# Terascale-All-sensing-Research-Studio/MOV-SLAM

Measured on AMD Instinct MI355X. Metric: local-BA iterations/sec (50 KF x 20k MapPoint window), higher is better.
Workload: dtype f64; 1 GPU; LocalBundleAdjustment 50 KF + 10 fixed x 20000 MapPoints, E=110510 mono edges, Huber on, 10 LM iterations (cfg3, seed 1003); one window per GPU; parallelism=1 window

## Files before the change

### mov-slam_amd/csrc/structure.cpp

```cpp
#include "structure.h"

#include <algorithm>
#include <cstdlib>
#include <cstring>

namespace movba {

void reset_structure(Structure& s, int NP, int P, int E)
{
    s.nfree = 0; s.npairs = 0; s.nitems = 0; s.max_degree = 0; s.nentries = 0; s.already_grouped = true; s.n_fixed = 0; s.n_agg = 0; s.reordered = false;
    s.free_pose.clear(); s.pair_i.clear(); s.pair_j.clear(); s.items.clear(); s.sched.clear(); s.sched_per_xcd = 0; s.row_ent.clear();
    s.cblk_g.clear(); s.cblk_h.clear(); s.cblk_ptr.clear(); s.cblk_ent.clear(); s.ent_i.clear(); s.ent_j.clear(); s.ent_l.clear(); s.E_free = 0;
    s.NP = NP; s.P = P; s.E = E;
}

void index_poses(const uint8_t* pose_fixed, Structure& s)
{
    const int NP = s.NP;
    s.hidx.assign(NP, -1);
    std::vector<int32_t>& pstart = s.pose_slot0;
    pstart.assign(NP + 1, -1);
    int run = 0;
    for (int i = 0; i < NP; ++i) {
        if (pose_fixed[i]) { s.n_fixed++; continue; }
        if (s.pose_edges[i] > 0) { s.hidx[i] = s.nfree++; s.free_pose.push_back(i); pstart[i] = run; run += s.pose_edges[i]; }
    }
// ... 86 lines not shown
                --pos;
            }
            fe_h[pos] = h; fe_g[pos] = g;
            if (pos > base && fe_h[pos - 1] == h) return MOVBA_ERR_ARG;
            if (pos + 1 < fe_h.size() && fe_h[pos + 1] == h) return MOVBA_ERR_ARG;
        }
        fe_start[l + 1] = (int32_t)fe_h.size();
    }
    return MOVBA_OK;
}

int finish_pairs(Structure& s, const int32_t* cnt)
{
    const int nf = s.nfree;
    s.pid.assign((size_t)nf * (size_t)nf, -1);
    s.pair_i.clear(); s.pair_j.clear();
    for (int i = 0; i < nf; ++i) { s.pid[(size_t)i * nf + i] = i; s.pair_i.push_back(i); s.pair_j.push_back(i); }
    for (int i = 0; i < nf; ++i)
        for (int j = i + 1; j < nf; ++j)
            if (cnt[(size_t)i * nf + j] > 0) {
                s.pid[(size_t)i * nf + j] = (int32_t)s.pair_i.size();
                s.pair_i.push_back(i); s.pair_j.push_back(j);
            }
    s.npairs = (int)s.pair_i.size();
    s.pair_ptr.assign(s.npairs + 1, 0);
    for (int p = 0; p < s.npairs; ++p) s.pair_ptr[p + 1] = s.pair_ptr[p] + cnt[(size_t)s.pair_i[p] * nf + s.pair_j[p]];
    s.nentries = s.pair_ptr[s.npairs];
    if (s.nentries > (int64_t)0x7fffffff) return MOVBA_ERR_ARG;
    if (nf > 0 && s.pair_ptr[nf] != (int64_t)s.E_free) return MOVBA_ERR_ARG;

    s.items.clear();
    s.pair_item_start.assign(s.npairs + 1, 0);
    for (int p = 0; p < s.npairs; ++p) {
        const int64_t cap = p < nf ? kSchurChunkDiag : kSchurChunk, len = s.pair_ptr[p + 1] - s.pair_ptr[p];
        const int64_t parts = (len + cap - 1) / cap;
        const int64_t chunk = parts > 0 ? ((len + parts - 1) / parts + 3) / 4 * 4 : cap;
        s.pair_item_start[p] = (int32_t)s.items.size();
        for (int64_t b = s.pair_ptr[p]; b < s.pair_ptr[p + 1]; b += chunk)
            s.items.push_back(Item{ p, (int32_t)b, (int32_t)std::min<int64_t>(b + chunk, s.pair_ptr[p + 1]), p < nf ? 1 : 0 });
    }
    s.pair_item_start[s.npairs] = (int32_t)s.items.size();
    s.nitems = (int)s.items.size();

    {
        const int ipw = kSchurWaves / kSchurWPI;
        std::vector<int32_t>& order = s.tmp_order;
        order.resize(s.nitems);
        {
            int n = 0, od = nf < s.npairs ? s.pair_item_start[nf] : s.nitems;
            for (int i = 0; i < nf; ++i) {
                for (int k = s.pair_item_start[i]; k < s.pair_item_start[i + 1]; ++k) order[n++] = k;
                while (od < s.nitems && s.pair_i[s.items[od].pair] == i) order[n++] = od++;
            }
        }
        auto weight = [&](int k) { const Item& it = s.items[k]; return (int64_t)(it.end - it.begin) * (it.diag ? 3 : 2) + 128; };
        int64_t total = 0;
        for (int k = 0; k < s.nitems; ++k) total += weight(k);
        std::vector<uint64_t>& key = s.tmp_key;
        key.resize(s.nitems);
        int seg_begin[9];
        {
            int64_t acc = 0; int x = 0;
            seg_begin[0] = 0;
            for (int n = 0; n < s.nitems; ++n) {
                while (x < 7 && acc >= (total * (x + 1)) / 8) seg_begin[++x] = n;
                const int64_t wgt = weight(order[n]);
                key[n] = ((uint64_t)(0x7fffffff - wgt) << 32) | (uint32_t)n;
                acc += wgt;
            }
            while (x < 8) seg_begin[++x] = s.nitems;
        }
#ifndef MOVBA_SCHUR_T1
#define MOVBA_SCHUR_T1 128
#define MOVBA_SCHUR_T2 256
#endif
#ifndef MOVBA_SCHUR_DW
#define MOVBA_SCHUR_DW 4
#endif
        auto waves_of = [&](int k) { const Item& it = s.items[k]; const int n = it.end - it.begin; return it.diag ? MOVBA_SCHUR_DW : (n > MOVBA_SCHUR_T2 ? 4 : (n > MOVBA_SCHUR_T1 ? 2 : 1)); };
        size_t longest = 1;
        for (int g = 0; g < 8; ++g) {
            std::sort(key.begin() + seg_begin[g], key.begin() + seg_begin[g + 1]);
            size_t slots = 0;
            for (int n = seg_begin[g]; n < seg_begin[g + 1]; ++n) {
                const size_t nw = (size_t)waves_of(order[(uint32_t)key[n]]);
                if ((slots & 3) + nw > 4) slots = (slots + 3) & ~(size_t)3;
                slots += nw;
            }
            longest = std::max(longest, (slots + 3) & ~(size_t)3);
        }
        (void)ipw;
        s.sched_per_xcd = (int)longest;
        s.sched.assign((size_t)8 * s.sched_per_xcd, SchedItem{ 0, 0, -1, 0, 0, -1, -1, 0 });
        for (int g = 0; g < 8; ++g) {
            size_t slots = 0;
            for (int n = seg_begin[g]; n < seg_begin[g + 1]; ++n) {
                const int item = order[(uint32_t)key[n]];
                const Item& it = s.items[item];
                const int nw = waves_of(item);
                if ((slots & 3) + (size_t)nw > 4) slots = (slots + 3) & ~(size_t)3;
                const int len = it.end - it.begin, epw = (len + nw - 1) / nw;
                for (int sub = 0; sub < nw; ++sub) {
                    const int wb = std::min(it.begin + sub * epw, it.end), we = std::min(wb + epw, it.end);
                    s.sched[(size_t)g * s.sched_per_xcd + slots + sub] = SchedItem{ wb, we, (item << 1) | (it.diag ? 1 : 0),
                                                                                   s.free_pose[s.pair_i[it.pair]], s.free_pose[s.pair_j[it.pair]], -1, -1, sub | (nw << 8) };
                }
                slots += (size_t)nw;
            }
        }
    }

    {
        s.row_ptr.assign(nf + 1, 0);
        for (int p = 0; p < s.npairs; ++p) {
            s.row_ptr[s.pair_i[p] + 1]++;
            if (p >= nf) s.row_ptr[s.pair_j[p] + 1]++;
        }
        for (int i = 0; i < nf; ++i) s.row_ptr[i + 1] = s.row_ptr[i] + ((s.row_ptr[i + 1] + 1) & ~1);
        s.row_ent.assign((size_t)s.row_ptr[nf], RowEnt{ -1, 0, 0, 0 });
        std::vector<int32_t>& cur = s.tmp_order;
        cur.assign(s.row_ptr.begin(), s.row_ptr.begin() + nf);
        for (int p = nf; p < s.npairs; ++p) s.row_ent[cur[s.pair_j[p]]++] = RowEnt{ p, s.pair_i[p], 1, 0 };
        for (int i = 0; i < nf; ++i) s.row_ent[cur[i]++] = RowEnt{ i, i, 0, 0 };
        for (int p = nf; p < s.npairs; ++p) s.row_ent[cur[s.pair_i[p]]++] = RowEnt{ p, s.pair_j[p], 0, 0 };
    }
    return MOVBA_OK;
}

bool covisibility_order(int nf, const int32_t* cnt, std::vector<int32_t>& new_of_old)
{
    new_of_old.resize(nf);
    for (int i = 0; i < nf; ++i) new_of_old[i] = i;
    if (nf < 3) return false;
    auto linked = [&](int a, int b) { return a == b ? false : (a < b ? cnt[(size_t)a * nf + b] : cnt[(size_t)b * nf + a]) > 0; };
    std::vector<int32_t> deg(nf, 0);
    for (int i = 0; i < nf; ++i) for (int j = i + 1; j < nf; ++j) if (cnt[(size_t)i * nf + j] > 0) { deg[i]++; deg[j]++; }
    auto envelope = [&](const std::vector<int32_t>& old_of_new) {
        int64_t env = 0;
        for (int r = 0; r < nf; ++r) {
            int first = r;
            for (int c = 0; c < r; ++c) if (linked(old_of_new[r], old_of_new[c])) { first = c; break; }
            env += r - first;
        }
        return env;
    };
    std::vector<int32_t> order, level(nf), queue;
    std::vector<uint8_t> placed(nf, 0);
    auto bfs = [&](int root, std::vector<int32_t>& out) {
        out.clear(); out.push_back(root);
        std::fill(level.begin(), level.end(), -1); level[root] = 0;
        for (size_t h = 0; h < out.size(); ++h) {
            const int v = out[h];
            const size_t first = out.size();
            for (int u = 0; u < nf; ++u) if (!placed[u] && level[u] < 0 && linked(v, u)) { level[u] = level[v] + 1; out.push_back(u); }
            std::sort(out.begin() + first, out.end(), [&](int a, int b) { return deg[a] != deg[b] ? deg[a] < deg[b] : a < b; });
        }
        return level[out.back()];
    };
    order.reserve(nf);
    for (;;) {
        int root = -1;
        for (int i = 0; i < nf; ++i) if (!placed[i] && (root < 0 || deg[i] < deg[root])) root = i;
        if (root < 0) break;
        for (int sweep = 0; sweep < 2; ++sweep) {
            const int depth = bfs(root, queue);
            int far = -1;
            for (int v : queue) if (level[v] == depth && (far < 0 || deg[v] < deg[far])) far = v;
            if (far == root) break;
            root = far;
        }
        bfs(root, queue);
        for (int v : queue) { placed[v] = 1; order.push_back(v); }
    }
    std::reverse(order.begin(), order.end());
    std::vector<int32_t> natural(nf);
    for (int i = 0; i < nf; ++i) natural[i] = i;
    const int64_t env_nat = envelope(natural), env_rcm = envelope(order);
    if (!(env_rcm * 5 < env_nat * 4)) return false;
    for (int k = 0; k < nf; ++k) new_of_old[order[k]] = k;
    return true;
}

void apply_pose_order(Structure& s, const std::vector<int32_t>& new_of_old, int32_t* cnt)
{
    const int nf = s.nfree;
    std::vector<int32_t> fp(nf);
    for (int h = 0; h < nf; ++h) fp[new_of_old[h]] = s.free_pose[h];
    s.free_pose = fp;
    for (int h = 0; h < nf; ++h) s.hidx[s.free_pose[h]] = h;
    int run = 0;
    for (int h = 0; h < nf; ++h) { s.pose_slot0[s.free_pose[h]] = run; run += s.pose_edges[s.free_pose[h]]; }
    if (cnt) {
        std::vector<int32_t> c2((size_t)nf * nf, 0);
        for (int i = 0; i < nf; ++i)
            for (int j = i; j < nf; ++j) {
                const int a = new_of_old[i], b = new_of_old[j];
                c2[(size_t)std::min(a, b) * nf + std::max(a, b)] = cnt[(size_t)i * nf + j];
            }
        std::memcpy(cnt, c2.data(), sizeof(int32_t) * c2.size());
    }
}

int build_structure(const movba_lba_desc& d, Structure& s)
{
    const int rc = build_basic(d, s);
    if (rc != MOVBA_OK) return rc;
    const int P = s.P, nf = s.nfree;

    std::vector<int32_t> fe_start, fe_h, fe_g;
    const int rf = free_lists(s, fe_start, fe_h, fe_g);
    if (rf != MOVBA_OK) return rf;
    std::vector<int32_t> cnt((size_t)nf * (size_t)nf, 0);
    for (int l = 0; l < P; ++l)
        for (int a = fe_start[l]; a < fe_start[l + 1]; ++a) {
            int32_t *row = &cnt[(size_t)fe_h[a] * nf];
            for (int b = a; b < fe_start[l + 1]; ++b) row[fe_h[b]]++;
        }
    if (nf <= 80 && !s.no_reorder) {
        std::vector<int32_t> new_of_old;
        if (covisibility_order(nf, cnt.data(), new_of_old)) {
            apply_pose_order(s, new_of_old, nullptr);
            build_slots(s);
            const int rf2 = free_lists(s, fe_start, fe_h, fe_g);
            if (rf2 != MOVBA_OK) return rf2;
            std::fill(cnt.begin(), cnt.end(), 0);
            for (int l = 0; l < P; ++l)
                for (int a = fe_start[l]; a < fe_start[l + 1]; ++a) {
                    int32_t *row = &cnt[(size_t)fe_h[a] * nf];
                    for (int b = a; b < fe_start[l + 1]; ++b) row[fe_h[b]]++;
                }
            s.reordered = true;
        }
    }
    const int rp = finish_pairs(s, cnt.data());
    if (rp != MOVBA_OK) return rp;
// ... 8 lines not shown
                const int32_t *prow = &s.pid[(size_t)fe_h[a] * nf];
                const int32_t ga = fe_g[a];
                for (int b = a + 1; b < fe_start[l + 1]; ++b) {
                    const int32_t pos = cur[prow[fe_h[b]]]++;
                    s.ent_i[pos] = s.slot[ga]; s.ent_j[pos] = s.slot[fe_g[b]]; s.ent_l[pos] = l;
                }
            }
    }
    return MOVBA_OK;
}

void build_coarse(Structure& s, const int32_t* agg_row0, int n_agg)
{
    const int nf = s.nfree, G = n_agg;
    s.n_agg = G;
    s.cblk_g.clear(); s.cblk_h.clear(); s.cblk_ent.clear(); s.cblk_ij.clear(); s.cblk_ptr.assign(1, 0);
    s.multi_pairs.clear();
    for (int p = nf; p < s.npairs; ++p)
        if (s.pair_item_start[p + 1] - s.pair_item_start[p] > 1) s.multi_pairs.push_back(p);
    std::vector<int32_t> agg_of(nf, 0);
    for (int g = 0; g < G; ++g)
        for (int i = agg_row0[g]; i < agg_row0[g + 1]; ++i) agg_of[i] = g;
    std::vector<std::vector<int32_t>> lists((size_t)G * G), ijs((size_t)G * G);
    for (int i = 0; i < nf; ++i)
        for (int e = s.row_ptr[i]; e < s.row_ptr[i + 1]; ++e)
            if (s.row_ent[e].block >= 0) {
                const size_t b = (size_t)agg_of[i] * G + agg_of[s.row_ent[e].col];
                const int pr = s.row_ent[e].block;
                const bool single = pr >= nf && s.pair_item_start[pr + 1] - s.pair_item_start[pr] == 1;
                const int src_idx = single ? s.pair_item_start[pr] : pr;
                lists[b].push_back((src_idx << 2) | (s.row_ent[e].transposed ? 2 : 0) | (single ? 1 : 0));
                ijs[b].push_back((i << 16) | s.row_ent[e].col);
            }
    for (int g = 0; g < G; ++g)
        for (int h = 0; h < G; ++h) {
            const std::vector<int32_t>& l = lists[(size_t)g * G + h];
            if (l.empty()) continue;
            s.cblk_g.push_back(g); s.cblk_h.push_back(h);
            s.cblk_ent.insert(s.cblk_ent.end(), l.begin(), l.end());
            s.cblk_ij.insert(s.cblk_ij.end(), ijs[(size_t)g * G + h].begin(), ijs[(size_t)g * G + h].end());
            s.cblk_ptr.push_back((int32_t)s.cblk_ent.size());
        }
}

}
```

### mov-slam_amd/csrc/structure.h

```cpp
#pragma once
#include <cstdint>
#include <vector>

#include "movba.h"

namespace movba {

struct Int2 { int32_t x, y; };
struct Int4 { int32_t x, y, z, w; };
struct Item { int32_t pair, begin, end, diag; };
struct SchedItem {
    int32_t begin, end, tag , pose_i, pose_j ;
    int32_t dst_a, dst_b;
    int32_t sub;
};
struct RowEnt { int32_t block, col, transposed, pad; };

struct Structure {
    int NP = 0, P = 0, E = 0, nfree = 0;
    int npairs = 0, nitems = 0, max_degree = 0;
    int64_t nentries = 0;
    bool already_grouped = true;
    bool reordered = false;
    bool no_reorder = false;
    int n_fixed = 0;
    std::vector<int32_t> hidx;
    std::vector<int32_t> free_pose;
    std::vector<int32_t> perm;
    std::vector<int32_t> tmp_order; std::vector<uint64_t> tmp_key;
    std::vector<int32_t> pose_edges, pose_slot0;
    std::vector<int32_t> pt_start;
    std::vector<int32_t> g_pose, g_point;
    const int32_t *gp = nullptr, *gl = nullptr;
    std::vector<int32_t> pair_i, pair_j;
    std::vector<int32_t> pair_item_start;
    std::vector<int64_t> pair_ptr;
    std::vector<int32_t> pid;
    std::vector<int32_t> slot;
    std::vector<int32_t> ent_i, ent_j, ent_l;
    int E_free = 0;
    std::vector<Item> items;
    std::vector<SchedItem> sched;
    int sched_per_xcd = 0;
    std::vector<int32_t> row_ptr;
// ... 15 lines not shown
#ifndef MOVBA_SCHUR_EPW_DIAG
#define MOVBA_SCHUR_EPW_DIAG 128
#endif
constexpr int kSchurWaves = MOVBA_SCHUR_WAVES;
constexpr int kSchurWPI = MOVBA_SCHUR_WPI;
constexpr int kSchurChunkDiag = MOVBA_SCHUR_EPW_DIAG * kSchurWPI;
constexpr int kSchurChunk = MOVBA_SCHUR_EPW * kSchurWPI;

int build_structure(const movba_lba_desc& d, Structure& s);
int build_basic(const movba_lba_desc& d, Structure& s, int32_t* rank_out = nullptr);
void reset_structure(Structure& s, int NP, int P, int E);
void index_poses(const uint8_t* pose_fixed, Structure& s);
void build_slots(Structure& s);
int finish_pairs(Structure& s, const int32_t* cnt);

bool covisibility_order(int nf, const int32_t* cnt, std::vector<int32_t>& new_of_old);
void apply_pose_order(Structure& s, const std::vector<int32_t>& new_of_old, int32_t* cnt );

}
```

### mov-slam_amd/csrc/upload.cpp

```cpp
#include <algorithm>
#include <cmath>
#include <cstring>
#include <vector>

#include "handle.h"
#include "kernels.h"

using namespace movba;

namespace {

inline void put(void *dst, const void *src, size_t bytes) { if (bytes) std::memcpy(dst, src, bytes); }

struct EdgeLayout {
    size_t gpose = 0, ptstart = 0, hidx = 0;
    size_t a_end = 0;
    size_t gpoint = 0, free_pose = 0, slot = 0;
    size_t base = 0;
    size_t raw_begin = 0, obs = 0, isig = 0, obsr = 0, pose0 = 0, point0 = 0, kcam = 0;
    size_t grouped_end = 0;
    size_t perm = 0;
    size_t max_end = 0;
    bool has_kcam = false;
};
// ... 88 lines not shown
    int32_t seq = 0;
    StructDev sd{};
    bool dev_structure = false, ent_packed = false, filled_early = false;
    bool scan_pending = false;
    bool sorted_structure = false;
    size_t s2_off = 0, s2_keys_in = 0, s2_keys_out = 0, s2_vals_in = 0, s2_tmp = 0, s2_tmp_bytes = 0;
    uint64_t fill_gen = 0;
    size_t noff = 0, o_ent = 0, o_slotpt = 0;
    size_t pair_begin = 0, hole = 0, h2d = 0, total = 0;
    size_t o_items = 0, o_sched = 0, o_pi = 0, o_pj = 0, o_pis = 0, o_rowptr = 0, o_rowent = 0, o_plan = 0;
    size_t o_cg = 0, o_ch = 0, o_cp = 0, o_ce = 0, o_cij = 0, o_multi = 0, o_pid = 0, o_prange = 0, o_dtp = 0, o_dtk = 0;
    size_t o_st[2][11] = {};
    size_t o_obspm = 0, o_obsrpm = 0, o_part = 0, o_blocks = 0, o_blocks_ov = 0, o_blocks_c = 0, o_aci = 0, o_acitag = 0;
    size_t o_bp = 0, o_xp = 0, o_scale = 0, o_hmax = 0, o_tick = 0, o_recd = 0, o_imgb = 0, o_ctrl = 0, o_chi2 = 0, o_outl = 0;
    size_t o_dtiles = 0, o_ddiag = 0, o_dfail = 0, o_dx = 0, o_dflags = 0, o_dcontrib = 0, o_dstamps = 0;
    std::vector<int32_t> lane_plan;
    int rec_slots = 1;
    size_t ncb = 0;
    int ntile = 0;
    bool dense_one = false, dense_stamps = false;
    double t0 = 0.0, lap_t = 0.0;
    bool lap_on = false;

    Upload(movba_handle *h_, const movba_lba_desc *d_) : h(h_), d(d_), NP(d_->n_poses), P(d_->n_points), E(d_->n_edges) {}
    ~Upload() { h->packer.wait(); if (direct_raw && !raw_synced) (void)hipStreamSynchronize(h->copy_stream); }

    const Structure &s() const { return h->st; }
    void lap(const char *what)
    {
        if (!lap_on) return;
        const double t = now_ms();
// ... 338 lines not shown
    if (!s().already_grouped) {
        { const int rw = join_helper(); if (rw) return rw; }
        HIP_TRY(hipStreamWaitEvent(h->stream, h->copy_event, 0));
        HIP_TRY(hipMemcpyAsync(h->arena + L.raw_begin, sg + L.raw_begin, edge_bytes - L.raw_begin, hipMemcpyHostToDevice, h->stream));
    }
    edge_b_queued = true;
    return MOVBA_OK;
}

int Upload::structure_on_host()
{
    const int rc = build_structure(*d, h->st);
    if (rc < 0) return rc;
    rank_mode = false;
    pack_b(false); edge_b_stale = true;
    noff = (size_t)(s().nentries - s().E_free);
    o_slotpt = c.take<int32_t>((size_t)s().E_free + 1);
    return MOVBA_OK;
}

int Upload::carve_scratch(bool basic)
{
    const int nchunks = (P + 63) / 64;
    Carver sc;
    so_cnt = sc.take<int32_t>(nbins); so_err = sc.take<int32_t>(4);
    so_pe = sc.take<int32_t>(basic ? NP : 0); so_info = sc.take<int32_t>(basic ? kBasicInfo : 0);
    so_ent0 = sc.take<int32_t>(nbins);
    so_cntw = sc.take<int32_t>(sorted_structure ? 0 : (size_t)nbins * nchunks);
    so_cntpt = sc.take<int32_t>(sorted_structure ? (size_t)P + 1 : 0);
    so_fixed = sc.take<uint8_t>(basic ? (size_t)NP + 4 : 0);
// ... 60 lines not shown
{
    int rc = carve_scratch(false); if (rc) return rc;
    HIP_TRY(hipMemsetAsync(h->scratch.p + so_cnt, 0, so_err + 16 - so_cnt, h->stream));
    rc = launch_counts(); if (rc) return rc;
    lap("edge H2D + count launches");
    return after_counts();
}

int Upload::after_counts()
{
    int32_t *cnt = misc();
    if (!dev_first) { const int rc = wait_for_counts(); if (rc) return rc; }
    if (cnt[nbins] != 0) return MOVBA_ERR_ARG;
    lap("wait for the pair counts");
    if (!h->st.no_reorder) {
        std::vector<int32_t> new_of_old;
        if (covisibility_order(nf, cnt, new_of_old)) {
            apply_pose_order(h->st, new_of_old, cnt);
            h->st.reordered = true;
            std::memcpy(sg + L.hidx, s().hidx.data(), sizeof(int32_t) * NP);
            std::memcpy(sg + L.base, s().pose_slot0.data(), sizeof(int32_t) * NP);
            std::memcpy(sg + L.free_pose, s().free_pose.data(), sizeof(int32_t) * nf);
            HIP_TRY(hipMemcpyAsync(h->arena + L.hidx, sg + L.hidx, sizeof(int32_t) * NP, hipMemcpyHostToDevice, h->stream));
            if (dev_first) {
                HIP_TRY(hipMemcpyAsync(h->arena + L.base, sg + L.base, sizeof(int32_t) * NP, hipMemcpyHostToDevice, h->stream));
                HIP_TRY(hipMemcpyAsync(h->arena + L.free_pose, sg + L.free_pose, sizeof(int32_t) * nf, hipMemcpyHostToDevice, h->stream));
            } else edge_b_stale = true;
            HIP_TRY(hipMemsetAsync(h->scratch.p + so_cnt, 0, so_err + 16 - so_cnt, h->stream));
            HIP_TRY(launch_struct_count(sd, h->stream));
            HIP_TRY(launch_struct_counts_out(sd, nullptr, 0, h->stream));
            HIP_TRY(launch_struct_scan(sd, h->stream));
            scan_pending = false;
// ... 147 lines not shown
        const bool forced = h->opt.solver == 2 || (h->opt.solver == 0 && band_env == 1);
        const bool off = h->opt.solver == 3 || h->opt.solver == 1 || (h->opt.solver == 0 && band_env == 0);
        const bool want = forced || (h->rows_kernel && est <= 130000.0);
        h->band = want && !off && band_supported(nf, bw);
    }
    if (h->rows_kernel && !h->band) build_coarse(h->st, h->pp.wave_row0, kPcgRowsThreads / 64);
    lap("pcg plan + coarse lists");
}

int Upload::lay_out_rest()
{
    pair_begin = c.off; hole = pair_begin - L.max_end;
    o_items = c.take<Item>((size_t)s().nitems + 1); o_sched = c.take<SchedItem>(s().sched.size() + 1);
    o_pi = c.take<int32_t>(s().npairs + 1); o_pj = c.take<int32_t>(s().npairs + 1); o_pis = c.take<int32_t>(s().npairs + 1);
    o_rowptr = c.take<int32_t>(nf + 1); o_rowent = c.take<RowEnt>(s().row_ent.size() + 1);
    lane_plan.clear();
    if (h->rows_kernel) {
        lane_plan.assign((size_t)kPcgRowsThreads * 12, -1);
        for (int wv = 0; wv < kPcgRowsThreads / 64; ++wv) {
            const int r0 = h->pp.wave_row0[wv], r1 = h->pp.wave_row0[wv + 1];
            const int P0 = s().row_ptr[r0] >> 1, P1 = s().row_ptr[r1] >> 1;
            for (int ln = 0; ln < 64 && P0 + ln < P1; ++ln)
                for (int k = 0; k < 2; ++k) {
                    const RowEnt &re = s().row_ent[2 * (P0 + ln) + k];
                    int32_t *pl = &lane_plan[((size_t)(wv * 64 + ln) * 3 + k) * 4];
                    if (re.block < 0) continue;
                    pl[0] = re.block; pl[1] = (re.col * 6) | (re.transposed ? (1 << 30) : 0);
                    pl[2] = s().pair_item_start[re.block]; pl[3] = s().pair_item_start[re.block + 1];
                }
            for (int ln = 0; ln < 64; ++ln) {
// ... 2 lines not shown
                if (ln >= 6 * (r1 - r0)) continue;
                const int bi = r0 + ln / 6;
                pl[0] = s().pair_item_start[bi]; pl[1] = s().pair_item_start[bi + 1]; pl[2] = s().row_ptr[bi]; pl[3] = s().row_ptr[bi + 1];
            }
        }
        for (int wv = 0; wv <= kPcgRowsThreads / 64; ++wv) h->pp.wave_ent0[wv] = s().row_ptr[h->pp.wave_row0[wv]];
        h->pp.nrowent = s().row_ptr[nf];
    }
    rec_slots = 1;
    for (int hh = 0; hh < nf; ++hh) rec_slots = std::max(rec_slots, (int)(s().pair_item_start[hh + 1] - s().pair_item_start[hh]));
    for (SchedItem &si : h->st.sched) {
        si.dst_a = -1; si.dst_b = -1;
        if (si.tag >= 0 && (si.tag & 1)) { const Item &it = s().items[(size_t)(si.tag >> 1)]; si.dst_a = it.pair * rec_slots + ((si.tag >> 1) - s().pair_item_start[it.pair]); }
    }
    if (h->rows_kernel && !h->pp.overflow) {
        std::vector<int32_t> slot_of_item((size_t)s().nitems, -1);
        for (size_t q = 0; q < s().sched.size(); ++q)
            if (s().sched[q].tag >= 0 && (s().sched[q].sub & 0xff) == 0) slot_of_item[(size_t)(s().sched[q].tag >> 1)] = (int32_t)q;
        for (int t = 0; t < kPcgRowsThreads; ++t)
            for (int k = 0; k < 2; ++k) {
                const int32_t *pl = &lane_plan[((size_t)t * 3 + k) * 4];
                if (pl[0] < nf || pl[3] - pl[2] != 1) continue;
                SchedItem &si = h->st.sched[(size_t)slot_of_item[(size_t)pl[2]]];
                const int32_t dst = 36 * k * kPcgRowsThreads + t;
                if ((pl[1] >> 30) & 1) si.dst_b = dst; else si.dst_a = dst;
            }
    }
    ncb = s().cblk_g.size();
    o_plan = c.take<int32_t>(lane_plan.size() + 4);
    o_cg = c.take<int32_t>(ncb + 1); o_ch = c.take<int32_t>(ncb + 1); o_cp = c.take<int32_t>(ncb + 2); o_ce = c.take<int32_t>(s().cblk_ent.size() + 1);
    o_cij = c.take<int32_t>(s().cblk_ij.size() + 1); o_multi = c.take<int32_t>(s().multi_pairs.size() + 1);
    o_pid = c.take<int32_t>((size_t)nf * nf + 1);
    ntile = dense_ntile(nf);
// ... 6 lines not shown
    if (!dev_structure) o_ent = c.take<int32_t>(ent_words());
    h2d = c.off;
    if (!state_carved) carve_state();
    const size_t part_stride = ((size_t)s().nitems * kPartStride + 31) / 32 * 32;
    o_part = c.take<double>(part_stride + 1); o_blocks = c.take<double>((size_t)s().npairs * 36 + 1);
    o_recd = c.take<double>((size_t)nf * rec_slots * 48 + 2); o_imgb = c.take<double>((size_t)72 * kPcgRowsThreads);
    o_blocks_ov = c.take<double>(h->rows_kernel && h->pp.overflow ? s().row_ent.size() * 36 + 2 : 2);
    o_blocks_c = c.take<double>((size_t)s().npairs * 36 + 1);
    o_dtiles = c.take<double>(dense_tiles_doubles(nf)); o_ddiag = c.take<double>((size_t)ntile * kDenseNB * kDenseNB + 1); o_dfail = c.take<int32_t>(4);
    o_dx = c.take<double>((size_t)ntile * kDenseNB + 1);
    o_dflags = c.take<uint32_t>(dense_one ? (size_t)dense_flag_words(ntile) : 8);
    o_dcontrib = c.take<double>(dense_one ? (size_t)ntile * ntile * kDenseNB : 1);
    dense_stamps = process_switches().dense_stamps;
    o_dstamps = c.take<unsigned long long>(dense_one && dense_stamps ? 6 * h->dplan.tasks.size() : 1);
    total = c.off;

    if (total > h->arena_cap || h2d - hole + misc_bytes > h->stage_cap) { const int rw = join_helper(); if (rw) return rw; }
    int rc = ensure_arena(h, total); if (rc) return rc;
    if (dev_first && (h->arena_gen != arena_gen_at_edge_copy || h2d - hole + misc_bytes > h->stage_cap)) return kRetryClassic;
    if (h->arena_gen != arena_gen_at_edge_copy) {
        HIP_TRY(hipMemcpyAsync(h->arena, sg, edge_bytes, hipMemcpyHostToDevice, h->stream));
        aim_struct_dev();
    }
    if (h2d - hole + misc_bytes > h->stage_cap) {
        rc = ensure_stage(h, h2d - hole + misc_bytes); if (rc) return rc;
        sg = h->stage;
        pack_edges(true);
    }
    return MOVBA_OK;
}
// ... 5 lines not shown
        if (ent_packed) {
            unsigned long long *e64 = reinterpret_cast<unsigned long long *>(eh);
            for (size_t k = 0; k < noff; ++k) e64[k] = ent_pack(s().ent_i[k], s().ent_j[k], s().ent_l[k]);
        } else {
            put(eh, s().ent_i.data(), sizeof(int32_t) * noff); put(eh + noff, s().ent_j.data(), sizeof(int32_t) * noff);
            put(eh + 2 * noff, s().ent_l.data(), sizeof(int32_t) * noff);
        }
    }
    put(sp(o_items), s().items.data(), sizeof(Item) * (size_t)s().nitems);
    put(sp(o_sched), s().sched.data(), sizeof(SchedItem) * s().sched.size());
    put(sp(o_pi), s().pair_i.data(), sizeof(int32_t) * s().npairs);
    put(sp(o_pj), s().pair_j.data(), sizeof(int32_t) * s().npairs);
    put(sp(o_pis), s().pair_item_start.data(), sizeof(int32_t) * (s().npairs + 1));
    put(sp(o_rowptr), s().row_ptr.data(), sizeof(int32_t) * (nf + 1));
    put(sp(o_rowent), s().row_ent.data(), sizeof(RowEnt) * s().row_ent.size());
    if (!lane_plan.empty()) put(sp(o_plan), lane_plan.data(), sizeof(int32_t) * lane_plan.size());
    put(sp(o_cg), s().cblk_g.data(), sizeof(int32_t) * ncb);
    put(sp(o_ch), s().cblk_h.data(), sizeof(int32_t) * ncb);
    put(sp(o_cp), s().cblk_ptr.data(), sizeof(int32_t) * s().cblk_ptr.size());
    put(sp(o_ce), s().cblk_ent.data(), sizeof(int32_t) * s().cblk_ent.size());
    put(sp(o_cij), s().cblk_ij.data(), sizeof(int32_t) * s().cblk_ij.size());
    put(sp(o_multi), s().multi_pairs.data(), sizeof(int32_t) * s().multi_pairs.size());
    put(sp(o_pid), s().pid.data(), sizeof(int32_t) * (size_t)nf * nf);
    if (dense_one) {
        put(sp(o_dtp), h->dplan.task_ptr.data(), sizeof(int32_t) * h->dplan.task_ptr.size());
        put(sp(o_dtk), h->dplan.tasks.data(), sizeof(DenseTask) * h->dplan.tasks.size());
        int32_t *pr = reinterpret_cast<int32_t *>(sp(o_prange));
        for (size_t q = 0; q < (size_t)nf * nf; ++q) {
            const int32_t pair = s().pid[q];
            pr[2 * q] = pair >= 0 ? s().pair_item_start[pair] : 0;
            pr[2 * q + 1] = pair >= 0 ? s().pair_item_start[pair + 1] : 0;
        }
    }
    lap("carve + pack pair region");
}

int Upload::send_pairs()
{
    const double t2 = now_ms();
    h->prof.structure_ms += (t2 - t0) - upload_host_ms;
    if (h2d - pair_begin <= (size_t)1 << 20) {
        IngestArgs ia{};
        ia.seg[0] = IngestSeg{ h->stage_dev + L.max_end, h->arena + pair_begin, ((h2d - pair_begin) + 3) & ~(size_t)3 };
        ia.nseg = 1; ia.counter = nullptr; ia.wait_for = 0;
        HIP_TRY(launch_ingest(ia, h->stream));
    } else
        HIP_TRY(hipMemcpyAsync(h->arena + pair_begin, sg + L.max_end, h2d - pair_begin, hipMemcpyHostToDevice, h->stream));
    if (!(filled_early && fill_gen == h->arena_gen)) { const int rq = queue_slots_and_fill(); if (rq) return rq; }
    { const int rw = join_helper(); if (rw) return rw; }
// ... 153 lines not shown
```

Baseline: 9478 LM iterations/s.

## Speed up host-side structure build with radix sort, adjacency-list RCM and reused scratch

```diff
diff --git a/mov-slam_amd/csrc/structure.cpp b/mov-slam_amd/csrc/structure.cpp
--- a/mov-slam_amd/csrc/structure.cpp
+++ b/mov-slam_amd/csrc/structure.cpp
@@ -9,7 +9,7 @@
 void reset_structure(Structure& s, int NP, int P, int E)
 {
     s.nfree = 0; s.npairs = 0; s.nitems = 0; s.max_degree = 0; s.nentries = 0; s.already_grouped = true; s.n_fixed = 0; s.n_agg = 0; s.reordered = false;
-    s.free_pose.clear(); s.pair_i.clear(); s.pair_j.clear(); s.items.clear(); s.sched.clear(); s.sched_per_xcd = 0; s.row_ent.clear();
+    s.free_pose.clear(); s.pair_i.clear(); s.pair_j.clear(); s.items.clear(); s.sched_per_xcd = 0; s.row_ent.clear();
     s.cblk_g.clear(); s.cblk_h.clear(); s.cblk_ptr.clear(); s.cblk_ent.clear(); s.ent_i.clear(); s.ent_j.clear(); s.ent_l.clear(); s.E_free = 0;
     s.NP = NP; s.P = P; s.E = E;
 }
@@ -126,61 +126,102 @@
 {
     const int nf = s.nfree;
     s.pid.assign((size_t)nf * (size_t)nf, -1);
-    s.pair_i.clear(); s.pair_j.clear();
-    for (int i = 0; i < nf; ++i) { s.pid[(size_t)i * nf + i] = i; s.pair_i.push_back(i); s.pair_j.push_back(i); }
-    for (int i = 0; i < nf; ++i)
-        for (int j = i + 1; j < nf; ++j)
-            if (cnt[(size_t)i * nf + j] > 0) {
-                s.pid[(size_t)i * nf + j] = (int32_t)s.pair_i.size();
-                s.pair_i.push_back(i); s.pair_j.push_back(j);
-            }
-    s.npairs = (int)s.pair_i.size();
-    s.pair_ptr.assign(s.npairs + 1, 0);
+    s.pair_i.resize((size_t)nf * (nf + 1) / 2); s.pair_j.resize((size_t)nf * (nf + 1) / 2);
+    {
+        int32_t *pi = s.pair_i.data(), *pj = s.pair_j.data(), *pid = s.pid.data();
+        for (int i = 0; i < nf; ++i) { pid[(size_t)i * nf + i] = i; pi[i] = i; pj[i] = i; }
+        int np = nf;
+        for (int i = 0; i < nf; ++i) {
+            const int32_t *row = cnt + (size_t)i * nf;
+            int32_t *prow = pid + (size_t)i * nf;
+            for (int j = i + 1; j < nf; ++j)
+                if (row[j] > 0) { prow[j] = np; pi[np] = i; pj[np] = j; ++np; }
+        }
+        s.npairs = np;
+        s.pair_i.resize(np); s.pair_j.resize(np);
+    }
+    s.pair_ptr.resize(s.npairs + 1);
+    s.pair_ptr[0] = 0;
     for (int p = 0; p < s.npairs; ++p) s.pair_ptr[p + 1] = s.pair_ptr[p] + cnt[(size_t)s.pair_i[p] * nf + s.pair_j[p]];
     s.nentries = s.pair_ptr[s.npairs];
     if (s.nentries > (int64_t)0x7fffffff) return MOVBA_ERR_ARG;
     if (nf > 0 && s.pair_ptr[nf] != (int64_t)s.E_free) return MOVBA_ERR_ARG;
 
-    s.items.clear();
-    s.pair_item_start.assign(s.npairs + 1, 0);
-    for (int p = 0; p < s.npairs; ++p) {
-        const int64_t cap = p < nf ? kSchurChunkDiag : kSchurChunk, len = s.pair_ptr[p + 1] - s.pair_ptr[p];
-        const int64_t parts = (len + cap - 1) / cap;
-        const int64_t chunk = parts > 0 ? ((len + parts - 1) / parts + 3) / 4 * 4 : cap;
-        s.pair_item_start[p] = (int32_t)s.items.size();
-        for (int64_t b = s.pair_ptr[p]; b < s.pair_ptr[p + 1]; b += chunk)
-            s.items.push_back(Item{ p, (int32_t)b, (int32_t)std::min<int64_t>(b + chunk, s.pair_ptr[p + 1]), p < nf ? 1 : 0 });
-    }
-    s.pair_item_start[s.npairs] = (int32_t)s.items.size();
-    s.nitems = (int)s.items.size();
-
-    {
-        const int ipw = kSchurWaves / kSchurWPI;
-        std::vector<int32_t>& order = s.tmp_order;
-        order.resize(s.nitems);
+    s.pair_item_start.resize(s.npairs + 1);
+    {
+        const int64_t *pp = s.pair_ptr.data();
+        auto chunk_of = [&](int p, int64_t len) {
+            const int64_t cap = p < nf ? kSchurChunkDiag : kSchurChunk;
+            const int64_t parts = (len + cap - 1) / cap;
+            return parts > 0 ? ((len + parts - 1) / parts + 3) / 4 * 4 : cap;
+        };
+        int32_t *pis = s.pair_item_start.data();
+        int ni = 0;
+        for (int p = 0; p < s.npairs; ++p) {
+            const int64_t cap = p < nf ? kSchurChunkDiag : kSchurChunk, len = pp[p + 1] - pp[p];
+            pis[p] = ni;
+            if (len <= cap) ni += len > 0; else { const int64_t chunk = chunk_of(p, len); ni += (int)((len + chunk - 1) / chunk); }
+        }
+        pis[s.npairs] = ni;
+        s.items.resize(ni);
+        Item *it = s.items.data();
+        for (int p = 0; p < s.npairs; ++p) {
+            const int n = pis[p + 1] - pis[p], diag = p < nf ? 1 : 0;
+            if (n == 1) { it[pis[p]] = Item{ p, (int32_t)pp[p], (int32_t)pp[p + 1], diag }; continue; }
+            if (n == 0) continue;
+            const int64_t chunk = chunk_of(p, pp[p + 1] - pp[p]);
+            int k = pis[p];
+            for (int64_t b = pp[p]; b < pp[p + 1]; b += chunk) it[k++] = Item{ p, (int32_t)b, (int32_t)std::min<int64_t>(b + chunk, pp[p + 1]), diag };
+        }
+        s.nitems = ni;
+    }
+
+    {
+        const int ni = s.nitems;
+        const Item *items = s.items.data();
+        s.tmp_order.resize(ni);
+        s.tmp_sorted.resize((size_t)4 * ni);
+        int32_t *order = s.tmp_order.data(), *wgt = s.tmp_sorted.data(), *seg_of = wgt + ni, *by_w = wgt + 2 * (size_t)ni, *final_n = wgt + 3 * (size_t)ni;
         {
-            int n = 0, od = nf < s.npairs ? s.pair_item_start[nf] : s.nitems;
+            int n = 0, od = nf < s.npairs ? s.pair_item_start[nf] : ni;
             for (int i = 0; i < nf; ++i) {
                 for (int k = s.pair_item_start[i]; k < s.pair_item_start[i + 1]; ++k) order[n++] = k;
-                while (od < s.nitems && s.pair_i[s.items[od].pair] == i) order[n++] = od++;
-            }
-        }
-        auto weight = [&](int k) { const Item& it = s.items[k]; return (int64_t)(it.end - it.begin) * (it.diag ? 3 : 2) + 128; };
+                while (od < ni && s.pair_i[items[od].pair] == i) order[n++] = od++;
+            }
+        }
         int64_t total = 0;
-        for (int k = 0; k < s.nitems; ++k) total += weight(k);
-        std::vector<uint64_t>& key = s.tmp_key;
-        key.resize(s.nitems);
+        int wmax = 0, wmin = 0x7fffffff;
+        for (int n = 0; n < ni; ++n) {
+            const Item& it = items[order[n]];
+            const int w = (it.end - it.begin) * (it.diag ? 3 : 2) + 128;
+            wgt[n] = w; total += w; wmax = std::max(wmax, w); wmin = std::min(wmin, w);
+        }
         int seg_begin[9];
         {
             int64_t acc = 0; int x = 0;
             seg_begin[0] = 0;
-            for (int n = 0; n < s.nitems; ++n) {
+            for (int n = 0; n < ni; ++n) {
                 while (x < 7 && acc >= (total * (x + 1)) / 8) seg_begin[++x] = n;
-                const int64_t wgt = weight(order[n]);
-                key[n] = ((uint64_t)(0x7fffffff - wgt) << 32) | (uint32_t)n;
-                acc += wgt;
-            }
-            while (x < 8) seg_begin[++x] = s.nitems;
+                seg_of[n] = x;
+                acc += wgt[n];
+            }
+            while (x < 8) seg_begin[++x] = ni;
+        }
+        {
+            const unsigned span = ni > 0 ? (unsigned)(wmax - wmin) : 0u;
+            int32_t *src = final_n, *dst = by_w;
+            for (int n = 0; n < ni; ++n) src[n] = n;
+            for (unsigned shift = 0; shift == 0 || (span >> shift) != 0; shift += 7) {
+                int32_t hist[129] = {};
+                for (int n = 0; n < ni; ++n) hist[(((unsigned)(wmax - wgt[n]) >> shift) & 127u) + 1]++;
+                for (int b = 0; b < 128; ++b) hist[b + 1] += hist[b];
+                for (int k = 0; k < ni; ++k) { const int n = src[k]; dst[hist[((unsigned)(wmax - wgt[n]) >> shift) & 127u]++] = n; }
+                std::swap(src, dst);
+            }
+            if (src != by_w) std::memcpy(by_w, src, sizeof(int32_t) * (size_t)ni);
+            int cur[8];
+            for (int g = 0; g < 8; ++g) cur[g] = seg_begin[g];
+            for (int k = 0; k < ni; ++k) { const int n = by_w[k]; final_n[cur[seg_of[n]]++] = n; }
         }
 #ifndef MOVBA_SCHUR_T1
 #define MOVBA_SCHUR_T1 128
@@ -189,36 +230,38 @@
 #ifndef MOVBA_SCHUR_DW
 #define MOVBA_SCHUR_DW 4
 #endif
-        auto waves_of = [&](int k) { const Item& it = s.items[k]; const int n = it.end - it.begin; return it.diag ? MOVBA_SCHUR_DW : (n > MOVBA_SCHUR_T2 ? 4 : (n > MOVBA_SCHUR_T1 ? 2 : 1)); };
+        auto waves_of = [&](int k) { const Item& it = items[k]; const int n = it.end - it.begin; return it.diag ? MOVBA_SCHUR_DW : (n > MOVBA_SCHUR_T2 ? 4 : (n > MOVBA_SCHUR_T1 ? 2 : 1)); };
         size_t longest = 1;
-        for (int g = 0; g < 8; ++g) {
-            std::sort(key.begin() + seg_begin[g], key.begin() + seg_begin[g + 1]);
-            size_t slots = 0;
-            for (int n = seg_begin[g]; n < seg_begin[g + 1]; ++n) {
-                const size_t nw = (size_t)waves_of(order[(uint32_t)key[n]]);
-                if ((slots & 3) + nw > 4) slots = (slots + 3) & ~(size_t)3;
-                slots += nw;
-            }
-            longest = std::max(longest, (slots + 3) & ~(size_t)3);
-        }
-        (void)ipw;
-        s.sched_per_xcd = (int)longest;
-        s.sched.assign((size_t)8 * s.sched_per_xcd, SchedItem{ 0, 0, -1, 0, 0, -1, -1, 0 });
         for (int g = 0; g < 8; ++g) {
             size_t slots = 0;
             for (int n = seg_begin[g]; n < seg_begin[g + 1]; ++n) {
-                const int item = order[(uint32_t)key[n]];
-                const Item& it = s.items[item];
+                const size_t nw = (size_t)waves_of(order[final_n[n]]);
+                if ((slots & 3) + nw > 4) slots = (slots + 3) & ~(size_t)3;
+                slots += nw;
+            }
+            longest = std::max(longest, (slots + 3) & ~(size_t)3);
+        }
+        s.sched_per_xcd = (int)longest;
+        s.sched.resize((size_t)8 * s.sched_per_xcd);
+        const SchedItem padding{ 0, 0, -1, 0, 0, -1, -1, 0 };
+        const int32_t *fp = s.free_pose.data(), *pi = s.pair_i.data(), *pj = s.pair_j.data();
+        for (int g = 0; g < 8; ++g) {
+            SchedItem *seg = s.sched.data() + (size_t)g * s.sched_per_xcd;
+            size_t slots = 0;
+            for (int n = seg_begin[g]; n < seg_begin[g + 1]; ++n) {
+                const int item = order[final_n[n]];
+                const Item& it = items[item];
                 const int nw = waves_of(item);
-                if ((slots & 3) + (size_t)nw > 4) slots = (slots + 3) & ~(size_t)3;
+                if ((slots & 3) + (size_t)nw > 4) while (slots & 3) seg[slots++] = padding;
                 const int len = it.end - it.begin, epw = (len + nw - 1) / nw;
+                const int32_t tag = (item << 1) | (it.diag ? 1 : 0), pose_i = fp[pi[it.pair]], pose_j = fp[pj[it.pair]];
                 for (int sub = 0; sub < nw; ++sub) {
                     const int wb = std::min(it.begin + sub * epw, it.end), we = std::min(wb + epw, it.end);
-                    s.sched[(size_t)g * s.sched_per_xcd + slots + sub] = SchedItem{ wb, we, (item << 1) | (it.diag ? 1 : 0),
-                                                                                   s.free_pose[s.pair_i[it.pair]], s.free_pose[s.pair_j[it.pair]], -1, -1, sub | (nw << 8) };
+                    seg[slots + sub] = SchedItem{ wb, we, tag, pose_i, pose_j, -1, -1, sub | (nw << 8) };
                 }
                 slots += (size_t)nw;
             }
+            while (slots < (size_t)s.sched_per_xcd) seg[slots++] = padding;
         }
     }
 
@@ -241,53 +284,79 @@
 
 bool covisibility_order(int nf, const int32_t* cnt, std::vector<int32_t>& new_of_old)
 {
+    OrderScratch scratch;
+    return covisibility_order(nf, cnt, new_of_old, scratch);
+}
+
+bool covisibility_order(int nf, const int32_t* cnt, std::vector<int32_t>& new_of_old, OrderScratch& sc)
+{
     new_of_old.resize(nf);
     for (int i = 0; i < nf; ++i) new_of_old[i] = i;
     if (nf < 3) return false;
-    auto linked = [&](int a, int b) { return a == b ? false : (a < b ? cnt[(size_t)a * nf + b] : cnt[(size_t)b * nf + a]) > 0; };
-    std::vector<int32_t> deg(nf, 0);
-    for (int i = 0; i < nf; ++i) for (int j = i + 1; j < nf; ++j) if (cnt[(size_t)i * nf + j] > 0) { deg[i]++; deg[j]++; }
-    auto envelope = [&](const std::vector<int32_t>& old_of_new) {
+    sc.deg.assign(nf, 0); sc.adj_ptr.resize(nf + 1); sc.by_deg.resize(nf); sc.level.resize(nf); sc.pos.resize(nf);
+    sc.tmp.assign(nf + 1, 0); sc.placed.assign(nf, 0);
+    int32_t *deg = sc.deg.data(), *adj_ptr = sc.adj_ptr.data(), *by_deg = sc.by_deg.data(), *level = sc.level.data(), *pos = sc.pos.data(), *cur = sc.tmp.data();
+    uint8_t *placed = sc.placed.data();
+    for (int i = 0; i < nf; ++i) {
+        const int32_t *row = cnt + (size_t)i * nf;
+        for (int j = i + 1; j < nf; ++j) if (row[j] > 0) { deg[i]++; deg[j]++; }
+    }
+    adj_ptr[0] = 0;
+    for (int i = 0; i < nf; ++i) { adj_ptr[i + 1] = adj_ptr[i] + deg[i]; cur[deg[i] + 1]++; }
+    for (int d = 0; d < nf; ++d) cur[d + 1] += cur[d];
+    for (int i = 0; i < nf; ++i) by_deg[cur[deg[i]]++] = i;
+    sc.adj.resize((size_t)adj_ptr[nf]);
+    int32_t *adj = sc.adj.data();
+    for (int i = 0; i < nf; ++i) cur[i] = adj_ptr[i];
+    for (int k = 0; k < nf; ++k) {
+        const int u = by_deg[k];
+        for (int v = 0; v < u; ++v) if (cnt[(size_t)v * nf + u] > 0) adj[cur[v]++] = u;
+        const int32_t *row = cnt + (size_t)u * nf;
+        for (int v = u + 1; v < nf; ++v) if (row[v] > 0) adj[cur[v]++] = u;
+    }
+    auto envelope = [&]() {
         int64_t env = 0;
-        for (int r = 0; r < nf; ++r) {
-            int first = r;
-            for (int c = 0; c < r; ++c) if (linked(old_of_new[r], old_of_new[c])) { first = c; break; }
-            env += r - first;
+        for (int v = 0; v < nf; ++v) {
+            int first = pos[v];
+            for (int e = adj_ptr[v]; e < adj_ptr[v + 1]; ++e) first = std::min(first, pos[adj[e]]);
+            env += pos[v] - first;
         }
         return env;
     };
-    std::vector<int32_t> order, level(nf), queue;
-    std::vector<uint8_t> placed(nf, 0);
-    auto bfs = [&](int root, std::vector<int32_t>& out) {
-        out.clear(); out.push_back(root);
-        std::fill(level.begin(), level.end(), -1); level[root] = 0;
-        for (size_t h = 0; h < out.size(); ++h) {
-            const int v = out[h];
-            const size_t first = out.size();
-            for (int u = 0; u < nf; ++u) if (!placed[u] && level[u] < 0 && linked(v, u)) { level[u] = level[v] + 1; out.push_back(u); }
-            std::sort(out.begin() + first, out.end(), [&](int a, int b) { return deg[a] != deg[b] ? deg[a] < deg[b] : a < b; });
-        }
-        return level[out.back()];
+    sc.queue.resize(nf); sc.order.resize(nf);
+    int32_t *queue = sc.queue.data(), *order = sc.order.data();
+    int nq = 0, nplaced = 0;
+    auto bfs = [&](int root) {
+        nq = 0; queue[nq++] = root;
+        std::fill(level, level + nf, -1); level[root] = 0;
+        for (int h = 0; h < nq; ++h) {
+            const int v = queue[h];
+            for (int e = adj_ptr[v]; e < adj_ptr[v + 1]; ++e) {
+                const int u = adj[e];
+                if (!placed[u] && level[u] < 0) { level[u] = level[v] + 1; queue[nq++] = u; }
+            }
+        }
+        return level[queue[nq - 1]];
     };
-    order.reserve(nf);
     for (;;) {
         int root = -1;
         for (int i = 0; i < nf; ++i) if (!placed[i] && (root < 0 || deg[i] < deg[root])) root = i;
         if (root < 0) break;
         for (int sweep = 0; sweep < 2; ++sweep) {
-            const int depth = bfs(root, queue);
+            const int depth = bfs(root);
             int far = -1;
-            for (int v : queue) if (level[v] == depth && (far < 0 || deg[v] < deg[far])) far = v;
+            for (int k = 0; k < nq; ++k) { const int v = queue[k]; if (level[v] == depth && (far < 0 || deg[v] < deg[far])) far = v; }
             if (far == root) break;
             root = far;
         }
-        bfs(root, queue);
-        for (int v : queue) { placed[v] = 1; order.push_back(v); }
-    }
-    std::reverse(order.begin(), order.end());
-    std::vector<int32_t> natural(nf);
-    for (int i = 0; i < nf; ++i) natural[i] = i;
-    const int64_t env_nat = envelope(natural), env_rcm = envelope(order);
+        bfs(root);
+        for (int k = 0; k < nq; ++k) { placed[queue[k]] = 1; order[nplaced++] = queue[k]; }
+    }
+    std::reverse(order, order + nf);
+    for (int i = 0; i < nf; ++i) pos[i] = i;
+    const int64_t env_nat = envelope();
+    for (int k = 0; k < nf; ++k) pos[order[k]] = k;
+    const int64_t env_rcm = envelope();
     if (!(env_rcm * 5 < env_nat * 4)) return false;
     for (int k = 0; k < nf; ++k) new_of_old[order[k]] = k;
     return true;
@@ -296,14 +365,16 @@
 void apply_pose_order(Structure& s, const std::vector<int32_t>& new_of_old, int32_t* cnt)
 {
     const int nf = s.nfree;
-    std::vector<int32_t> fp(nf);
+    std::vector<int32_t>& fp = s.order_scratch.tmp;
+    fp.resize(nf);
     for (int h = 0; h < nf; ++h) fp[new_of_old[h]] = s.free_pose[h];
-    s.free_pose = fp;
+    s.free_pose.assign(fp.begin(), fp.end());
     for (int h = 0; h < nf; ++h) s.hidx[s.free_pose[h]] = h;
     int run = 0;
     for (int h = 0; h < nf; ++h) { s.pose_slot0[s.free_pose[h]] = run; run += s.pose_edges[s.free_pose[h]]; }
     if (cnt) {
-        std::vector<int32_t> c2((size_t)nf * nf, 0);
+        std::vector<int32_t>& c2 = s.order_scratch.adj;
+        c2.assign((size_t)nf * nf, 0);
         for (int i = 0; i < nf; ++i)
             for (int j = i; j < nf; ++j) {
                 const int a = new_of_old[i], b = new_of_old[j];
@@ -329,8 +400,8 @@
             for (int b = a; b < fe_start[l + 1]; ++b) row[fe_h[b]]++;
         }
     if (nf <= 80 && !s.no_reorder) {
-        std::vector<int32_t> new_of_old;
-        if (covisibility_order(nf, cnt.data(), new_of_old)) {
+        std::vector<int32_t>& new_of_old = s.new_of_old;
+        if (covisibility_order(nf, cnt.data(), new_of_old, s.order_scratch)) {
             apply_pose_order(s, new_of_old, nullptr);
             build_slots(s);
             const int rf2 = free_lists(s, fe_start, fe_h, fe_g);
@@ -369,33 +440,44 @@
 {
     const int nf = s.nfree, G = n_agg;
     s.n_agg = G;
-    s.cblk_g.clear(); s.cblk_h.clear(); s.cblk_ent.clear(); s.cblk_ij.clear(); s.cblk_ptr.assign(1, 0);
     s.multi_pairs.clear();
     for (int p = nf; p < s.npairs; ++p)
         if (s.pair_item_start[p + 1] - s.pair_item_start[p] > 1) s.multi_pairs.push_back(p);
-    std::vector<int32_t> agg_of(nf, 0);
+    s.tmp_hist.assign((size_t)nf + (size_t)G * G, 0);
+    int32_t *agg_of = s.tmp_hist.data(), *cur = agg_of + nf;
     for (int g = 0; g < G; ++g)
         for (int i = agg_row0[g]; i < agg_row0[g + 1]; ++i) agg_of[i] = g;
-    std::vector<std::vector<int32_t>> lists((size_t)G * G), ijs((size_t)G * G);
-    for (int i = 0; i < nf; ++i)
-        for (int e = s.row_ptr[i]; e < s.row_ptr[i + 1]; ++e)
-            if (s.row_ent[e].block >= 0) {
-                const size_t b = (size_t)agg_of[i] * G + agg_of[s.row_ent[e].col];
-                const int pr = s.row_ent[e].block;
-                const bool single = pr >= nf && s.pair_item_start[pr + 1] - s.pair_item_start[pr] == 1;
-                const int src_idx = single ? s.pair_item_start[pr] : pr;
-                lists[b].push_back((src_idx << 2) | (s.row_ent[e].transposed ? 2 : 0) | (single ? 1 : 0));
-                ijs[b].push_back((i << 16) | s.row_ent[e].col);
-            }
+    const RowEnt *row_ent = s.row_ent.data();
+    const int32_t *row_ptr = s.row_ptr.data(), *pis = s.pair_item_start.data();
+    for (int i = 0; i < nf; ++i) {
+        int32_t *crow = cur + (size_t)agg_of[i] * G;
+        for (int e = row_ptr[i]; e < row_ptr[i + 1]; ++e)
+            if (row_ent[e].block >= 0) crow[agg_of[row_ent[e].col]]++;
+    }
+    s.cblk_g.clear(); s.cblk_h.clear(); s.cblk_ptr.assign(1, 0);
+    int total = 0;
     for (int g = 0; g < G; ++g)
         for (int h = 0; h < G; ++h) {
-            const std::vector<int32_t>& l = lists[(size_t)g * G + h];
-            if (l.empty()) continue;
-            s.cblk_g.push_back(g); s.cblk_h.push_back(h);
-            s.cblk_ent.insert(s.cblk_ent.end(), l.begin(), l.end());
-            s.cblk_ij.insert(s.cblk_ij.end(), ijs[(size_t)g * G + h].begin(), ijs[(size_t)g * G + h].end());
-            s.cblk_ptr.push_back((int32_t)s.cblk_ent.size());
-        }
-}
-
-}
+            const int n = cur[(size_t)g * G + h];
+            cur[(size_t)g * G + h] = total;
+            if (n == 0) continue;
+            total += n;
+            s.cblk_g.push_back(g); s.cblk_h.push_back(h); s.cblk_ptr.push_back(total);
+        }
+    s.cblk_ent.resize(total); s.cblk_ij.resize(total);
+    int32_t *ent = s.cblk_ent.data(), *ij = s.cblk_ij.data();
+    for (int i = 0; i < nf; ++i) {
+        int32_t *crow = cur + (size_t)agg_of[i] * G;
+        for (int e = row_ptr[i]; e < row_ptr[i + 1]; ++e)
+            if (row_ent[e].block >= 0) {
+                const int pr = row_ent[e].block;
+                const bool single = pr >= nf && pis[pr + 1] - pis[pr] == 1;
+                const int src_idx = single ? pis[pr] : pr;
+                const int at = crow[agg_of[row_ent[e].col]]++;
+                ent[at] = (src_idx << 2) | (row_ent[e].transposed ? 2 : 0) | (single ? 1 : 0);
+                ij[at] = (i << 16) | row_ent[e].col;
+            }
+    }
+}
+
+}
diff --git a/mov-slam_amd/csrc/structure.h b/mov-slam_amd/csrc/structure.h
--- a/mov-slam_amd/csrc/structure.h
+++ b/mov-slam_amd/csrc/structure.h
@@ -16,6 +16,12 @@
 };
 struct RowEnt { int32_t block, col, transposed, pad; };
 
+#define MOVBA_LAYOUT_SCRATCH 1
+struct OrderScratch {
+    std::vector<int32_t> deg, by_deg, adj_ptr, adj, level, queue, order, pos, tmp;
+    std::vector<uint8_t> placed;
+};
+
 struct Structure {
     int NP = 0, P = 0, E = 0, nfree = 0;
     int npairs = 0, nitems = 0, max_degree = 0;
@@ -28,6 +34,9 @@
     std::vector<int32_t> free_pose;
     std::vector<int32_t> perm;
     std::vector<int32_t> tmp_order; std::vector<uint64_t> tmp_key;
+    std::vector<int32_t> tmp_sorted, tmp_hist;
+    OrderScratch order_scratch; std::vector<int32_t> new_of_old;
+    std::vector<int32_t> lane_plan, slot_of_item;
     std::vector<int32_t> pose_edges, pose_slot0;
     std::vector<int32_t> pt_start;
     std::vector<int32_t> g_pose, g_point;
@@ -73,6 +82,7 @@
 void build_slots(Structure& s);
 int finish_pairs(Structure& s, const int32_t* cnt);
 
+bool covisibility_order(int nf, const int32_t* cnt, std::vector<int32_t>& new_of_old, OrderScratch& scratch);
 bool covisibility_order(int nf, const int32_t* cnt, std::vector<int32_t>& new_of_old);
 void apply_pose_order(Structure& s, const std::vector<int32_t>& new_of_old, int32_t* cnt );
 
diff --git a/mov-slam_amd/csrc/upload.cpp b/mov-slam_amd/csrc/upload.cpp
--- a/mov-slam_amd/csrc/upload.cpp
+++ b/mov-slam_amd/csrc/upload.cpp
@@ -126,7 +126,6 @@
     size_t o_obspm = 0, o_obsrpm = 0, o_part = 0, o_blocks = 0, o_blocks_ov = 0, o_blocks_c = 0, o_aci = 0, o_acitag = 0;
     size_t o_bp = 0, o_xp = 0, o_scale = 0, o_hmax = 0, o_tick = 0, o_recd = 0, o_imgb = 0, o_ctrl = 0, o_chi2 = 0, o_outl = 0;
     size_t o_dtiles = 0, o_ddiag = 0, o_dfail = 0, o_dx = 0, o_dflags = 0, o_dcontrib = 0, o_dstamps = 0;
-    std::vector<int32_t> lane_plan;
     int rec_slots = 1;
     size_t ncb = 0;
     int ntile = 0;
@@ -495,6 +494,11 @@
     if (rc < 0) return rc;
     rank_mode = false;
     pack_b(false); edge_b_stale = true;
+    if (s().reordered) {
+        HIP_TRY(hipStreamSynchronize(h->stream));
+        put(sg + L.hidx, s().hidx.data(), sizeof(int32_t) * NP);
+        HIP_TRY(hipMemcpyAsync(h->arena + L.hidx, sg + L.hidx, sizeof(int32_t) * NP, hipMemcpyHostToDevice, h->stream));
+    }
     noff = (size_t)(s().nentries - s().E_free);
     o_slotpt = c.take<int32_t>((size_t)s().E_free + 1);
     return MOVBA_OK;
@@ -585,8 +589,10 @@
     if (cnt[nbins] != 0) return MOVBA_ERR_ARG;
     lap("wait for the pair counts");
     if (!h->st.no_reorder) {
-        std::vector<int32_t> new_of_old;
-        if (covisibility_order(nf, cnt, new_of_old)) {
+        std::vector<int32_t> &new_of_old = h->st.new_of_old;
+        const bool renumber = covisibility_order(nf, cnt, new_of_old, h->st.order_scratch);
+        lap("covisibility order");
+        if (renumber) {
             apply_pose_order(h->st, new_of_old, cnt);
             h->st.reordered = true;
             std::memcpy(sg + L.hidx, s().hidx.data(), sizeof(int32_t) * NP);
@@ -764,6 +770,7 @@
     o_items = c.take<Item>((size_t)s().nitems + 1); o_sched = c.take<SchedItem>(s().sched.size() + 1);
     o_pi = c.take<int32_t>(s().npairs + 1); o_pj = c.take<int32_t>(s().npairs + 1); o_pis = c.take<int32_t>(s().npairs + 1);
     o_rowptr = c.take<int32_t>(nf + 1); o_rowent = c.take<RowEnt>(s().row_ent.size() + 1);
+    std::vector<int32_t> &lane_plan = h->st.lane_plan;
     lane_plan.clear();
     if (h->rows_kernel) {
         lane_plan.assign((size_t)kPcgRowsThreads * 12, -1);
@@ -796,9 +803,11 @@
         if (si.tag >= 0 && (si.tag & 1)) { const Item &it = s().items[(size_t)(si.tag >> 1)]; si.dst_a = it.pair * rec_slots + ((si.tag >> 1) - s().pair_item_start[it.pair]); }
     }
     if (h->rows_kernel && !h->pp.overflow) {
-        std::vector<int32_t> slot_of_item((size_t)s().nitems, -1);
-        for (size_t q = 0; q < s().sched.size(); ++q)
-            if (s().sched[q].tag >= 0 && (s().sched[q].sub & 0xff) == 0) slot_of_item[(size_t)(s().sched[q].tag >> 1)] = (int32_t)q;
+        std::vector<int32_t> &slot_of_item = h->st.slot_of_item;
+        slot_of_item.assign((size_t)s().nitems, -1);
+        const SchedItem *sc = s().sched.data();
+        for (size_t q = 0, nq = s().sched.size(); q < nq; ++q)
+            if (sc[q].tag >= 0 && (sc[q].sub & 0xff) == 0) slot_of_item[(size_t)(sc[q].tag >> 1)] = (int32_t)q;
         for (int t = 0; t < kPcgRowsThreads; ++t)
             for (int k = 0; k < 2; ++k) {
                 const int32_t *pl = &lane_plan[((size_t)t * 3 + k) * 4];
@@ -835,6 +844,7 @@
     dense_stamps = process_switches().dense_stamps;
     o_dstamps = c.take<unsigned long long>(dense_one && dense_stamps ? 6 * h->dplan.tasks.size() : 1);
     total = c.off;
+    lap("lay out the rest");
 
     if (total > h->arena_cap || h2d - hole + misc_bytes > h->stage_cap) { const int rw = join_helper(); if (rw) return rw; }
     int rc = ensure_arena(h, total); if (rc) return rc;
@@ -870,7 +880,7 @@
     put(sp(o_pis), s().pair_item_start.data(), sizeof(int32_t) * (s().npairs + 1));
     put(sp(o_rowptr), s().row_ptr.data(), sizeof(int32_t) * (nf + 1));
     put(sp(o_rowent), s().row_ent.data(), sizeof(RowEnt) * s().row_ent.size());
-    if (!lane_plan.empty()) put(sp(o_plan), lane_plan.data(), sizeof(int32_t) * lane_plan.size());
+    put(sp(o_plan), s().lane_plan.data(), sizeof(int32_t) * s().lane_plan.size());
     put(sp(o_cg), s().cblk_g.data(), sizeof(int32_t) * ncb);
     put(sp(o_ch), s().cblk_h.data(), sizeof(int32_t) * ncb);
     put(sp(o_cp), s().cblk_ptr.data(), sizeof(int32_t) * s().cblk_ptr.size());
@@ -882,13 +892,14 @@
         put(sp(o_dtp), h->dplan.task_ptr.data(), sizeof(int32_t) * h->dplan.task_ptr.size());
         put(sp(o_dtk), h->dplan.tasks.data(), sizeof(DenseTask) * h->dplan.tasks.size());
         int32_t *pr = reinterpret_cast<int32_t *>(sp(o_prange));
-        for (size_t q = 0; q < (size_t)nf * nf; ++q) {
-            const int32_t pair = s().pid[q];
-            pr[2 * q] = pair >= 0 ? s().pair_item_start[pair] : 0;
-            pr[2 * q + 1] = pair >= 0 ? s().pair_item_start[pair + 1] : 0;
+        std::memset(pr, 0, sizeof(int32_t) * 2 * (size_t)nf * nf);
+        const int32_t *pi = s().pair_i.data(), *pj = s().pair_j.data(), *pis = s().pair_item_start.data();
+        for (int p = 0; p < s().npairs; ++p) {
+            const size_t q = (size_t)pi[p] * nf + pj[p];
+            pr[2 * q] = pis[p]; pr[2 * q + 1] = pis[p + 1];
         }
     }
-    lap("carve + pack pair region");
+    lap("pack pair region");
 }
 
 int Upload::send_pairs()
```

Result: no change. 9424 LM iterations/s (-0.6%).
